# Maxwell-Zhao/RoboSimGS

Measured on AMD Instinct MI355X. Metric: frames/sec + ms/frame (fwd, fwd+bwd) at 1M Gaussians 1920x1080, higher is better.
Workload: dtype f32

## Files before the change

robosimgs_amd/csrc/build.py:

```python
from __future__ import annotations

import hashlib
import os
import shutil
import subprocess
import sys
from concurrent.futures import ThreadPoolExecutor

HERE = os.path.dirname(os.path.abspath(__file__))
SOURCES = ["api.hip", "projection.hip", "sort.hip", "binning.hip", "tile_sort.hip", "raster_fwd.hip",
           "raster_bwd.hip", "backward.hip", "composite.hip", "points.hip", "loss.hip", "transform.hip", "frame.hip"]
HEADERS = ["mgs_common.h", "mgs_math.h", "raster_common.h", "sh_staging.h", "tile_rect.h", "tile_order.h",
           "../../include/mgs.h"]
LIB = os.path.join(HERE, "libmgs.so")
DEBUG_LIB = os.path.join(HERE, "libmgs_debug.so")
HOOK_SOURCES = ["raster_fwd.hip", "sort.hip"]
OBJ_DIR = os.path.join(HERE, "build")
FLAGS = ["--offload-arch=gfx950", "-O3", "-std=c++17", "-fPIC", "-munsafe-fp-atomics",
         "-fno-slp-vectorize", "-Wall", "-Wno-unused-function"] + os.environ.get("MGS_EXTRA_FLAGS", "").split()


PER_SOURCE_FLAGS = {
    "raster_bwd.hip": os.environ.get("MGS_RASTER_BWD_FLAGS", "").split(),
    "raster_fwd.hip": os.environ.get("MGS_RASTER_FWD_FLAGS", "").split(),
    "tile_sort.hip": os.environ.get("MGS_TILE_SORT_FLAGS", "").split(),
    "binning.hip": os.environ.get("MGS_BINNING_FLAGS", "").split(),
}


def _hipcc() -> str:
    for c in (os.environ.get("HIPCC"), shutil.which("hipcc"), "/opt/rocm/bin/hipcc"):
        if c and os.path.exists(c):
            return c
    raise RuntimeError("hipcc not found; libmgs.so cannot be built")


def _stamp() -> str:
    h = hashlib.sha256((" ".join(FLAGS) + repr(sorted(PER_SOURCE_FLAGS.items()))).encode())
    for f in SOURCES + HEADERS:
        p = os.path.join(HERE, f)
        if os.path.exists(p):
            with open(p, "rb") as fh:
                h.update(fh.read())
    return h.hexdigest()


def _code_only(text: str) -> str:
    out, i, n = [], 0, len(text)
    while i < n:
        c = text[i]
        if c in "\"'":
            j = i + 1
            while j < n and text[j] != c:
                j += 2 if text[j] == "\\" else 1
            out.append(text[i:j + 1])
            i = j + 1
        elif text.startswith("//", i):
            j = text.find("\n", i)
            i = n if j < 0 else j
        elif text.startswith("/*", i):
            j = text.find("*/", i + 2)
            i = n if j < 0 else j + 2
            out.append(" ")
        else:
            out.append(c)
            i += 1
    return " ".join("".join(out).split())


def current_stamp() -> str:
    h = hashlib.sha256((" ".join(FLAGS) + repr(sorted(PER_SOURCE_FLAGS.items()))).encode())
    for f in SOURCES + HEADERS:
        p = os.path.join(HERE, f)
        if os.path.exists(p):
            with open(p, "r", encoding="utf-8", errors="replace") as fh:
                h.update(_code_only(fh.read()).encode())
    return h.hexdigest()


def build(force: bool = False, verbose: bool = False) -> str:
    stamp_file = os.path.join(OBJ_DIR, "stamp")
    stamp = _stamp()
    if (not force and os.path.exists(LIB) and os.path.exists(DEBUG_LIB) and os.path.exists(stamp_file)
            and open(stamp_file).read() == stamp):
        return LIB
    os.makedirs(OBJ_DIR, exist_ok=True)
    hipcc = _hipcc()
    srcs = [s for s in SOURCES if os.path.exists(os.path.join(HERE, s))]

    def compile_one(job) -> str:
        src, hooks = job
        obj = os.path.join(OBJ_DIR, src.replace(".hip", ".dbg.o" if hooks else ".o"))
        cmd = [hipcc, *FLAGS, *PER_SOURCE_FLAGS.get(src, []), *(["-DMGS_DEBUG_HOOKS"] if hooks else []), "-c",
               os.path.join(HERE, src), "-o", obj]
        if verbose:
            print(" ".join(cmd), flush=True)
        r = subprocess.run(cmd, capture_output=True, text=True)
        if r.returncode != 0:
            raise RuntimeError(f"hipcc failed on {src}:\n{r.stderr}")
# ... 21 lines not shown
```

robosimgs_amd/csrc/raster_bwd.hip:

```cpp
#include <algorithm>
#include <type_traits>

#include "raster_common.h"
#include "tile_order.h"

namespace mgs {
namespace {

template <int CHT, bool WIDE>
struct BwdEntry {
  float4 geo0;
  float4 geo1;
  float4 feat[(CHT + 3) / 4];
  float4 geo2;
  float4 geo3[WIDE ? 1 : 0];
};

template <int CHT>
struct BwdPixel {
  float T;
  float bv;
  float v_c[CHT];
  int last;
};

template <int CHT>
struct GaussGrad {
  float s, s_x, s_y, s_xx, s_xy, s_yy, a_x, a_y;
  float v_f[CHT];
};

template <int CHT, bool ABSGRAD, bool SAFE = false>
__device__ __forceinline__ void grad_pixel(BwdPixel<CHT>& px, GaussGrad<CHT>& gg, const PixelPoly& pp,
                                           float mx, float my, float ca, float cb,
                                           float cc, float A, float B, float C, float q0, float q1, float q2,
                                           const float* feat, int idx, int& any) {
  float ov = __builtin_amdgcn_exp2f(pair_power_poly(pp, q0, q1, q2, A, B, C));
  float alpha = SAFE ? ov : fminf(kAlphaMax, ov);
  bool valid = idx <= px.last && alpha >= kAlphaMin;
  if (!SAFE) valid = valid && pair_power_sign(mx - pp.x, my - pp.y, A, B, C) <= 0.f;
  if (ballot(valid) == 0ull) return;
  any = 1;
  float a_eff = valid ? alpha : 0.f;
  bool grad_geo = valid && ov <= kAlphaMax;
  float ov_eff = SAFE ? a_eff : (grad_geo ? ov : 0.f);
  float ra = __builtin_amdgcn_rcpf(1.0f - a_eff);
  px.T *= ra;
  float fac = a_eff * px.T;
  float fv = feat[0] * px.v_c[0];
#pragma unroll
  for (int c = 1; c < CHT; ++c) fv = fmaf(feat[c], px.v_c[c], fv);
  float v_alpha = fmaf(-px.bv, ra, fv * px.T);
  asm volatile("" : "+v"(px.bv), "+v"(v_alpha));
  px.bv = fmaf(fv, fac, px.bv);
#pragma unroll
  for (int c = 0; c < CHT; ++c) gg.v_f[c] = fmaf(fac, px.v_c[c], gg.v_f[c]);
  float v_sigma = -ov_eff * v_alpha;
  gg.s += v_sigma;
  gg.s_x = fmaf(v_sigma, pp.x, gg.s_x);
  gg.s_y = fmaf(v_sigma, pp.y, gg.s_y);
  gg.s_xx = fmaf(v_sigma, pp.xx, gg.s_xx);
  gg.s_xy = fmaf(v_sigma, pp.xy, gg.s_xy);
  gg.s_yy = fmaf(v_sigma, pp.yy, gg.s_yy);
  if (ABSGRAD) {
    float p = v_sigma * (mx - pp.x), q = v_sigma * (my - pp.y);
    gg.a_x += fabsf(fmaf(cb, q, ca * p));
    gg.a_y += fabsf(fmaf(cc, q, cb * p));
  }
}

__device__ __forceinline__ void moments_to_mean(float mx, float my, float s, float s_x, float s_y, float s_xx,
                                                float s_xy, float s_yy, float& P, float& Q, float& Vaa, float& Vab,
                                                float& Vbb) {
  P = fmaf(mx, s, -s_x);
  Q = fmaf(my, s, -s_y);
  Vaa = fmaf(mx, P, -fmaf(mx, s_x, -s_xx));
  Vab = fmaf(my, P, -fmaf(mx, s_y, -s_xy));
  Vbb = fmaf(my, Q, -fmaf(my, s_y, -s_yy));
}

__host__ __device__ constexpr int record_floats(int cht, bool absgrad) { return (6 + cht + (absgrad ? 2 : 0) + 3) / 4 * 4; }
__host__ __device__ constexpr int padded_channels(int channels) {
  return channels <= 4 ? channels : channels <= 8 ? 8 : channels <= 16 ? 16 : 32;
}

__device__ __forceinline__ void finish_geo(float ca, float cb, float cc, float& v_x, float& v_y,
                                           float& v_ca, float& v_cc) {
  const float s0 = v_x, s1 = v_y;
  v_x = fmaf(cb, s1, ca * s0);
  v_y = fmaf(cc, s1, cb * s0);
  v_ca *= 0.5f;
  v_cc *= 0.5f;
}

constexpr int kBwdMinWaves = 5;
constexpr int kBwdWgWaves = 1;
constexpr int kBwdXcdRun = 4;
#ifdef MGS_RASTER_BWD_TIMING
__device__ unsigned long long g_bwd_times[5 * 65536];
#endif
constexpr int kUnitClasses = 32;
struct UnitTables {
  uint32_t* counts;
  int4* whole;
  int4* part;
};
__host__ __device__ inline size_t unit_tables_bytes(int n_tiles, int shift, uint32_t capacity) {
  return 256 + (ckpt_units(capacity, n_tiles, shift) + (size_t)kUnitClasses * n_tiles) * sizeof(int4);
}
__device__ __forceinline__ UnitTables unit_tables(const int32_t* base, int n_tiles, int shift, uint32_t capacity) {
  UnitTables u;
  u.counts = reinterpret_cast<uint32_t*>(const_cast<int32_t*>(base));
  u.whole = reinterpret_cast<int4*>(const_cast<int32_t*>(base) + 64);
  u.part = u.whole + ckpt_units(capacity, n_tiles, shift);
  return u;
}

template <int CHT, bool ABSGRAD, bool RECORDS, bool SPLIT = false>
__device__ __forceinline__ void raster_bwd_unit(const int unit,
    const float* __restrict__ means2d, const float* __restrict__ conics,
    const float* __restrict__ feats, const float* __restrict__ opacities,
    const float4* __restrict__ splats, const float* __restrict__ background, int channels,
    int width, int height, int tile_w, int n_tiles, const int32_t* __restrict__ tile_offsets,
    const int32_t* __restrict__ flatten_ids, const float* __restrict__ alphas,
    const int32_t* __restrict__ last_ids, const float* __restrict__ v_render,
    const float* __restrict__ v_alphas, float* __restrict__ v_means2d,
    float* __restrict__ v_means2d_abs, float* __restrict__ v_conics,
    float* __restrict__ v_feats, float* __restrict__ v_opacities,
    const int4* __restrict__ pair_info, float* __restrict__ records,
    uint8_t* __restrict__ flags, uint32_t capacity, const float* __restrict__ expected_render,
    const int32_t* __restrict__ tile_order, const float* __restrict__ ckpt, int ckpt_shift,
    const int32_t* __restrict__ seg_table, const float* __restrict__ render_out, int splat_slots) {
  constexpr bool WIDE = ABSGRAD || !RECORDS;
  constexpr int NVR = 6 + CHT + (ABSGRAD ? 2 : 0);
  constexpr int kRedRows = !RECORDS ? 1 : (NVR > 8 && NVR <= 16) ? NVR : 8;
  __shared__ BwdEntry<CHT, WIDE> queues[kBwdWgWaves][kQueue];
  __shared__ float reds[kBwdWgWaves][kRedRows][64];
  BwdEntry<CHT, WIDE>* queue = queues[threadIdx.x >> 6];
  float (*red)[64] = reds[threadIdx.x >> 6];
  static_assert(!SPLIT || (RECORDS && CHT <= 4), "segments exist on the record path of up to 4 channels");
  constexpr int NQ = 4;
#ifdef MGS_RASTER_BWD_TIMING
  const unsigned long long t_enter = __builtin_amdgcn_s_memrealtime();
#endif
  int tile, seg = 0, seg_start = 0, seg_hi = 0;
  if constexpr (SPLIT) {
    const UnitTables ut = unit_tables(seg_table, n_tiles, ckpt_shift, capacity);
    uint32_t cnt[1 + kUnitClasses];
#pragma unroll
    for (int i = 0; i <= kUnitClasses; ++i) cnt[i] = ut.counts[i];
    const int4 e_whole = ut.whole[unit];
    int r = unit - (int)cnt[0], cls = -1, at = 0;
#pragma unroll
    for (int c = 0; c < kUnitClasses; ++c) {
      const int n = (int)cnt[1 + c];
      if (cls < 0 && r >= 0 && r < n) { cls = c; at = r; }
      if (r >= 0) r -= n;
    }
    if (r >= 0 && cls < 0) return;
    const int4 e = cls < 0 ? e_whole : ut.part[(size_t)cls * n_tiles + at];
    tile = e.x;
    seg = e.y;
    seg_start = e.z;
    seg_hi = e.w;
  } else {
    tile = tile_of_unit(unit, n_tiles, tile_order);
  }
  if (tile < 0) return;
  const unsigned lane = threadIdx.x & 63u;
  const int tx = tile % tile_w, ty = tile / tile_w;
  const float tile_x = (float)(tx * 16), tile_y = (float)(ty * 16);
  const int start = SPLIT ? seg_start : tile_offsets[tile], end = SPLIT ? seg_hi + 1 : tile_offsets[tile + 1];
  if (end <= start) return;
  const int lo = SPLIT ? start + (seg << ckpt_shift) : start;
  const int nxt = SPLIT ? lo + (1 << ckpt_shift) : end;
  if (RECORDS && capacity == 0u) return;
  const int ix = tx * 16 + (int)(lane & 7), iy = ty * 16 + (int)(lane >> 3);
  PixelPoly pq[NQ];
#pragma unroll
  for (int k = 0; k < NQ; ++k)
    pq[k] = pixel_poly((float)(lane & 7) - 7.5f + 8.f * (k & 1), (float)(int)(lane >> 3) - 7.5f + 8.f * (k >> 1));

  BwdPixel<CHT> st[NQ];
  int hi = -1;
  bool has_next = false;
  const float* cp = nullptr;
  if constexpr (SPLIT) {
    hi = seg_hi;
    if (hi < lo) return;
    has_next = hi >= nxt;
    cp = ckpt + ckpt_header_floats(n_tiles) + ckpt_unit(start, tile, seg + 1, ckpt_shift) * (size_t)(1 + channels) * 256 + lane;
    hi = min(hi, nxt - 1);
  }
  bool inside[NQ];
  float px_alpha[NQ], px_va[NQ], px_fin[NQ][CHT], px_ck[NQ][CHT + 1];
#pragma unroll
  for (int k = 0; k < NQ; ++k) {
    const int x = ix + 8 * (k & 1), y = iy + 8 * (k >> 1);
    inside[k] = x < width && y < height;
    const size_t p = inside[k] ? (size_t)y * width + x : 0;
    px_alpha[k] = inside[k] ? alphas[p] : 0.f;
    st[k].last = inside[k] ? last_ids[p] : -1;
    px_va[k] = (inside[k] && v_alphas) ? v_alphas[p] : 0.f;
    if (CHT == 4 && channels == 4) {
      const float4 v = inside[k] ? reinterpret_cast<const float4*>(v_render)[p] : make_float4(0.f, 0.f, 0.f, 0.f);
      st[k].v_c[0] = v.x; st[k].v_c[1 % CHT] = v.y; st[k].v_c[2 % CHT] = v.z; st[k].v_c[3 % CHT] = v.w;
    } else {
#pragma unroll
      for (int c = 0; c < CHT; ++c)
        st[k].v_c[c] = (inside[k] && c < channels) ? v_render[p * channels + c] : 0.f;
    }
    const float* frame = SPLIT ? (has_next ? render_out : expected_render) : expected_render;
#pragma unroll
    for (int c = 0; c < CHT; ++c) px_fin[k][c] = 0.f;
    if (frame && inside[k]) {
      if (CHT == 4 && channels == 4) {
        const float4 v = reinterpret_cast<const float4*>(frame)[p];
        px_fin[k][0] = v.x; px_fin[k][1 % CHT] = v.y; px_fin[k][2 % CHT] = v.z; px_fin[k][3 % CHT] = v.w;
      } else {
#pragma unroll
        for (int c = 0; c < CHT; ++c)
          if (c < channels && (SPLIT ? (has_next || c == channels - 1) : c == channels - 1)) px_fin[k][c] = frame[p * channels + c];
      }
    }
    if constexpr (SPLIT) {
#pragma unroll
      for (int c = 0; c <= CHT; ++c) px_ck[k][c] = (has_next && c <= channels) ? cp[256 * c + 64 * k] : 0.f;
    }
  }
#pragma unroll
  for (int k = 0; k < NQ; ++k) {
    st[k].T = 1.0f - px_alpha[k];
    float va = px_va[k];
    if (expected_render && inside[k]) {
      const float a = px_alpha[k], inv = 1.0f / fmaxf(a, 1e-10f);
#pragma unroll
      for (int c = 0; c < CHT; ++c)
        if (c == channels - 1) {
          const float v_ed = st[k].v_c[c];
          if (a > 1e-10f) va -= v_ed * px_fin[k][c] * inv;
          st[k].v_c[c] = v_ed * inv;
        }
    }
#pragma unroll
    for (int c = 0; c < CHT; ++c)
      if (background && c < channels) va -= background[c] * st[k].v_c[c];
    st[k].bv = -(st[k].T * va);
    if constexpr (SPLIT) {
      if (has_next && st[k].last >= nxt) {
        const float a = px_alpha[k], t_final = st[k].T;
        float behind = 0.f;
#pragma unroll
        for (int c = 0; c < CHT; ++c)
          if (c < channels) {
            float fin = px_fin[k][c];
            if (expected_render && c == channels - 1) fin *= fmaxf(a, 1e-10f);
            if (background) fin = fmaf(-t_final, background[c], fin);
            behind = fmaf(fin - px_ck[k][1 + c], st[k].v_c[c], behind);
          }
        st[k].bv += behind;
        st[k].T = px_ck[k][0];
      }
    } else {
      hi = max(hi, st[k].last);
    }
  }
  if constexpr (!SPLIT) {
#pragma unroll
    for (int d = 32; d >= 1; d >>= 1) hi = max(hi, __shfl_xor(hi, d));
    hi = min(hi, end - 1);
    if (hi < start) return;
  }
#ifdef MGS_RASTER_BWD_TIMING
  const unsigned long long t_begin = __builtin_amdgcn_s_memrealtime();
  unsigned long long n_walked = 0, n_pairs = 0;
#endif

  constexpr int NV = 6 + CHT + (ABSGRAD ? 2 : 0);
  constexpr int RSP = record_floats(CHT, ABSGRAD);
  auto rec_pos = [&](int j) { return j; };
  auto red_load = [&](float4& a0, float4& b0, float4& a1, float4& b1) {
    const int qv = (int)(lane >> 2), x = qv & 3;
    const float* q = &red[qv < NV ? qv : NV - 1][16 * (lane & 3)];
    a0 = *reinterpret_cast<const float4*>(q + 4 * x);
    b0 = *reinterpret_cast<const float4*>(q + 4 * (x ^ 1));
    a1 = *reinterpret_cast<const float4*>(q + 4 * (x ^ 2));
    b1 = *reinterpret_cast<const float4*>(q + 4 * (x ^ 3));
  };
  auto red_finish = [&](size_t rslot, const float4& a0, const float4& b0, const float4& a1, const float4& b1) {
    float t = (((a0.x + a0.y) + (a0.z + a0.w)) + ((b0.x + b0.y) + (b0.z + b0.w))) +
              (((a1.x + a1.y) + (a1.z + a1.w)) + ((b1.x + b1.y) + (b1.z + b1.w)));
    asm volatile("s_nop 1\n\tv_add_f32_dpp %0, %0, %0 quad_perm:[1,0,3,2] row_mask:0xf bank_mask:0xf\n\t"
                 "s_nop 1\n\tv_add_f32_dpp %0, %0, %0 quad_perm:[2,3,0,1] row_mask:0xf bank_mask:0xf" : "+v"(t));
    const float* rec = records + rslot * RSP;
    if ((lane & 3) == 0 && (int)(lane >> 2) < NV)
      asm volatile("global_store_dword %0, %1, %2" : : "v"((unsigned)(lane >> 2) * 4u), "v"(t), "s"(rec) : "memory");
    if (lane == 0) flags[rslot] = 1;
  };

  for (int q = (hi - start) / kQueue; q >= (lo - start) / kQueue; --q) {
    const int b = start + q * kQueue;
    unsigned live = 0;
#pragma unroll
    for (int k = 0; k < NQ; ++k)
      if (ballot(st[k].last >= b) != 0ull) live |= 1u << k;
    if (live == 0) continue;

    const int idx = b + (int)lane;
    unsigned qmask = 0;
    int g = 0;
    float2 xy = make_float2(0.f, 0.f);
    float ca = 1.f, cb = 0.f, cc = 1.f, op = 0.f;
    float pf[4] = {0.f, 0.f, 0.f, 0.f};
    uint32_t slot_base = 0u, slot_rect = 0u;
    const bool packed = CHT <= 4 && splats != nullptr;
    if (idx <= hi) {
      g = flatten_ids[idx];
      if (packed) {
        const float4 p0 = splats[3 * (size_t)g], p1 = splats[3 * (size_t)g + 1], p2 = splats[3 * (size_t)g + 2];
        xy = make_float2(p0.x, p0.y);
        ca = p0.z; cb = p0.w; cc = p1.x; op = p1.y;
        pf[0] = p1.z; pf[1] = p1.w; pf[2] = p2.x; pf[3] = p2.y;
        slot_base = __float_as_uint(p2.z); slot_rect = __float_as_uint(p2.w);
      } else {
        xy = reinterpret_cast<const float2*>(means2d)[g];
        ca = conics[3 * (size_t)g + 0];
        cb = conics[3 * (size_t)g + 1];
        cc = conics[3 * (size_t)g + 2];
        op = opacities[g];
      }
      qmask = quadrant_mask(xy.x, xy.y, ca, cb, cc, op, tile_x, tile_y);
      qmask &= live;
    }
    const unsigned long long keep = ballot(qmask != 0u);
    const int count = __popcll(keep);
#ifdef MGS_RASTER_BWD_TIMING
    n_walked += (unsigned long long)min(64, hi - b + 1);
    n_pairs += (unsigned long long)count;
#endif
    const bool all_safe = ballot(qmask != 0u && !entry_is_safe(ca, cb, cc, op)) == 0ull;
    if (qmask != 0u) {
      BwdEntry<CHT, WIDE>& e = queue[mask_rank(keep)];
      constexpr float kLog2e = 1.4426950408889634f;
      const float sA = -0.5f * kLog2e * ca, sB = -kLog2e * cb, sC = -0.5f * kLog2e * cc, L = __log2f(op);
      const float m_x = xy.x - (tile_x + 8.f), m_y = xy.y - (tile_y + 8.f);
      const PolyCoef pc = poly_coefs(m_x, m_y, sA, sB, sC, L);
      e.geo0 = make_float4(pc.q0, pc.q1, pc.q2, sA);
      e.geo1 = make_float4(sB, sC, __uint_as_float(qmask), __int_as_float(idx));
      int gid = g;
      if (RECORDS) {
        if (packed && splat_slots) {
          gid = (int)slot_base + (ty - (int)((slot_rect >> 10) & 1023u)) * (int)(slot_rect >> 20) + (tx - (int)(slot_rect & 1023u));
        } else {
          const int4 info = pair_info[g];
          gid = info.x + (ty - info.z) * (info.w & 0xffff) + (tx - info.y);
        }
      }
      e.geo2 = make_float4(__int_as_float(gid), m_x, m_y, L);
      if constexpr (WIDE) e.geo3[0] = make_float4(ca, cb, cc, 0.f);
      float f[((CHT + 3) / 4) * 4];
#pragma unroll
      for (int c = 0; c < ((CHT + 3) / 4) * 4; ++c)
        f[c] = (c < CHT && c < channels) ? (packed ? pf[c & 3] : feats[(size_t)g * channels + c]) : 0.f;
#pragma unroll
      for (int j = 0; j < (CHT + 3) / 4; ++j)
        e.feat[j] = make_float4(f[4 * j], f[4 * j + 1], f[4 * j + 2], f[4 * j + 3]);
    }
    __builtin_amdgcn_fence(__ATOMIC_RELEASE, "wavefront");
    __builtin_amdgcn_wave_barrier();
    __builtin_amdgcn_fence(__ATOMIC_ACQUIRE, "wavefront");

    auto walk = [&](auto safe_tag) {
    constexpr bool SAFE = decltype(safe_tag)::value;
    for (int j = count - 1; j >= 0; --j) {
      const BwdEntry<CHT, WIDE>& e = queue[j];
      const float4 g0 = e.geo0, g1 = e.geo1, g2 = e.geo2;
      float4 g3 = make_float4(0.f, 0.f, 0.f, 0.f);
      if constexpr (WIDE) g3 = e.geo3[0];
      float feat[CHT];
#pragma unroll
      for (int f = 0; f < (CHT + 3) / 4; ++f) {
        float4 v = e.feat[f];
        feat[4 * f] = v.x;
        if (4 * f + 1 < CHT) feat[4 * f + 1] = v.y;
        if (4 * f + 2 < CHT) feat[4 * f + 2] = v.z;
        if (4 * f + 3 < CHT) feat[4 * f + 3] = v.w;
      }
      const unsigned m = __builtin_amdgcn_readfirstlane(__float_as_uint(g1.z));
      const int gi = __float_as_int(g1.w);
      const int gid = __builtin_amdgcn_readfirstlane(__float_as_int(g2.x));
      GaussGrad<CHT> gg;
      gg.s = gg.s_x = gg.s_y = gg.s_xx = gg.s_xy = gg.s_yy = gg.a_x = gg.a_y = 0.f;
#pragma unroll
      for (int c = 0; c < CHT; ++c) gg.v_f[c] = 0.f;
      int any = 0;
#pragma unroll
      for (int k = 0; k < NQ; ++k) {
        if (m & (1u << k))
          grad_pixel<CHT, ABSGRAD, SAFE>(st[k], gg, pq[k], g2.y, g2.z, g3.x, g3.y, g3.z, g0.w, g1.x, g1.y,
                                         g0.x, g0.y, g0.z, feat, gi, any);
      }
      if (!any) continue;
      if constexpr (RECORDS) {
        if ((uint32_t)gid >= capacity) continue;
        const size_t rslot = (size_t)gid;
        float vals[NV];
        vals[0] = gg.s; vals[1] = gg.s_x; vals[2] = gg.s_y; vals[3] = gg.s_xx;
        vals[4] = gg.s_xy; vals[5] = gg.s_yy;
#pragma unroll
        for (int c = 0; c < CHT; ++c) vals[6 + c] = gg.v_f[c];
        if constexpr (ABSGRAD) { vals[6 + CHT] = gg.a_x; vals[7 + CHT] = gg.a_y; }
        int done = 0;
        if constexpr (NV > 8 && NV <= 16) {
#pragma unroll
          for (int i = 0; i < NV; ++i) red[i][lane] = vals[i];
          __builtin_amdgcn_fence(__ATOMIC_RELEASE, "wavefront");
          __builtin_amdgcn_wave_barrier();
          __builtin_amdgcn_fence(__ATOMIC_ACQUIRE, "wavefront");
          float4 a0, b0, a1, b1;
          red_load(a0, b0, a1, b1);
          red_finish(rslot, a0, b0, a1, b1);
          __builtin_amdgcn_wave_barrier();
          continue;
        }
        while (NV - done >= 8) {
#pragma unroll
          for (int i = 0; i < 8; ++i) red[i][lane] = vals[done + i];
          __builtin_amdgcn_fence(__ATOMIC_RELEASE, "wavefront");
          __builtin_amdgcn_wave_barrier();
          __builtin_amdgcn_fence(__ATOMIC_ACQUIRE, "wavefront");
          const float4* src = reinterpret_cast<const float4*>(&red[lane >> 3][(lane & 7) * 8]);
          const float4 a = src[0], b = src[1];
          float t = ((a.x + a.y) + (a.z + a.w)) + ((b.x + b.y) + (b.z + b.w));
          t += dpp_f(t, kDppXor1);
          t += dpp_f(t, kDppXor2);
          t += __int_as_float(__builtin_amdgcn_update_dpp(0, __float_as_int(t), 0x141, 0xf, 0xf, false));
          if ((lane & 7) == 0) {
            int pos = rec_pos(done + (int)(lane >> 3));
            if (pos >= 0) records[rslot * RSP + pos] = t;
          }
          __builtin_amdgcn_wave_barrier();
          done += 8;
        }
#define MGS_RS_CHUNK(V)                                                        \
        while (NV - done >= V) {                                               \
          float t = wave_reduce_scatter<V>(vals + done, lane);                 \
          int i = wave_reduce_scatter_index<V>(lane);                          \
          if (i >= 0) {                                                        \
            int pos = rec_pos(done + i);                                       \
            if (pos >= 0) records[rslot * RSP + pos] = t;                                        \
          }                                                                    \
          done += V;                                                           \
        }
        MGS_RS_CHUNK(4)
        MGS_RS_CHUNK(2)
        MGS_RS_CHUNK(1)
#undef MGS_RS_CHUNK
        if (lane == 0) flags[rslot] = 1;
      } else {
        const float ws = wave_reduce_to_lane63(gg.s), wx = wave_reduce_to_lane63(gg.s_x);
        const float wy = wave_reduce_to_lane63(gg.s_y), wxx = wave_reduce_to_lane63(gg.s_xx);
        const float wxy = wave_reduce_to_lane63(gg.s_xy), wyy = wave_reduce_to_lane63(gg.s_yy);
        float rx, ry, ra, rb, rc;
        moments_to_mean(g2.y, g2.z, ws, wx, wy, wxx, wxy, wyy, rx, ry, ra, rb, rc);
        const float ro = -ws * __builtin_amdgcn_exp2f(-g2.w);
        float rf[CHT];
#pragma unroll
        for (int c = 0; c < CHT; ++c) rf[c] = wave_reduce_to_lane63(gg.v_f[c]);
        float ax = 0.f, ay = 0.f;
        if (ABSGRAD) { ax = wave_reduce_to_lane63(gg.a_x); ay = wave_reduce_to_lane63(gg.a_y); }
        if (lane == 63) {
          finish_geo(g3.x, g3.y, g3.z, rx, ry, ra, rc);
          unsafeAtomicAdd(&v_means2d[2 * (size_t)gid + 0], rx);
          unsafeAtomicAdd(&v_means2d[2 * (size_t)gid + 1], ry);
          unsafeAtomicAdd(&v_conics[3 * (size_t)gid + 0], ra);
          unsafeAtomicAdd(&v_conics[3 * (size_t)gid + 1], rb);
          unsafeAtomicAdd(&v_conics[3 * (size_t)gid + 2], rc);
          unsafeAtomicAdd(&v_opacities[gid], ro);
#pragma unroll
          for (int c = 0; c < CHT; ++c)
            if (c < channels) unsafeAtomicAdd(&v_feats[(size_t)gid * channels + c], rf[c]);
          if (ABSGRAD) {
            unsafeAtomicAdd(&v_means2d_abs[2 * (size_t)gid + 0], ax);
            unsafeAtomicAdd(&v_means2d_abs[2 * (size_t)gid + 1], ay);
          }
        }
      }
    }
    };
    if (all_safe) walk(std::true_type{}); else walk(std::false_type{});
    __builtin_amdgcn_wave_barrier();
  }
#ifdef MGS_RASTER_BWD_TIMING
  if (lane == 0 && unit < 65536) {
    g_bwd_times[5 * unit + 0] = t_enter;
    g_bwd_times[5 * unit + 1] = t_begin;
    g_bwd_times[5 * unit + 2] = __builtin_amdgcn_s_memrealtime();
    g_bwd_times[5 * unit + 3] = n_walked;
    g_bwd_times[5 * unit + 4] = n_pairs;
  }
#endif
}

template <int CHT, bool ABSGRAD, bool RECORDS, bool SPLIT = false>
__global__ __launch_bounds__(64 * kBwdWgWaves, (CHT <= 4 && RECORDS && !ABSGRAD) ? kBwdMinWaves : 1) void raster_bwd_kernel(
    const float* __restrict__ means2d, const float* __restrict__ conics,
    const float* __restrict__ feats, const float* __restrict__ opacities,
    const float4* __restrict__ splats, const float* __restrict__ background, int channels,
    int width, int height, int tile_w, int n_tiles, const int32_t* __restrict__ tile_offsets,
    const int32_t* __restrict__ flatten_ids, const float* __restrict__ alphas,
    const int32_t* __restrict__ last_ids, const float* __restrict__ v_render,
    const float* __restrict__ v_alphas, float* __restrict__ v_means2d,
    float* __restrict__ v_means2d_abs, float* __restrict__ v_conics,
    float* __restrict__ v_feats, float* __restrict__ v_opacities,
    const int4* __restrict__ pair_info, float* __restrict__ records,
    uint8_t* __restrict__ flags, uint32_t capacity, const float* __restrict__ expected_render,
    const int32_t* __restrict__ tile_order, const float* __restrict__ ckpt, int ckpt_shift,
    const int32_t* __restrict__ seg_table, const float* __restrict__ render_out, int splat_slots) {
#define MGS_RB_ARGS means2d, conics, feats, opacities, splats, background, channels, width, height, tile_w, n_tiles, \
    tile_offsets, flatten_ids, alphas, last_ids, v_render, v_alphas, v_means2d, v_means2d_abs, v_conics, v_feats,    \
    v_opacities, pair_info, records, flags, capacity, expected_render, tile_order, ckpt, ckpt_shift, seg_table, render_out, splat_slots
  int unit = blockIdx.x * kBwdWgWaves + (int)(threadIdx.x >> 6);
  if constexpr (SPLIT && kBwdXcdRun > 1 && kBwdWgWaves == 1) {
    constexpr int R = kBwdXcdRun;
    const int b = unit, in = b % (8 * R);
    unit = b - in + (in & 7) * R + (in >> 3);
  }
  raster_bwd_unit<CHT, ABSGRAD, RECORDS, SPLIT>(unit, MGS_RB_ARGS);
#undef MGS_RB_ARGS
}

constexpr int kBigPairs = 256, kBigLists = 64, kBigWGs = 1024, kDiscoverPerThread = 16;
__host__ __device__ inline uint32_t big_list_room(uint32_t capacity) { return capacity / (uint32_t)kBigPairs + 1u; }
__host__ __device__ inline size_t big_lists_bytes(uint32_t capacity) { return (size_t)kBigLists * big_list_room(capacity) * sizeof(uint32_t); }

__device__ __forceinline__ void big_discover(int wg, int n, const int4* __restrict__ pair_info, uint32_t capacity,
                                             uint32_t* __restrict__ counts, uint32_t* __restrict__ items) {
  const int t = threadIdx.x;
  const uint32_t list = (uint32_t)(wg * 4 + (t >> 6)) % kBigLists, room = big_list_room(capacity);
  int4 info[kDiscoverPerThread];
#pragma unroll
  for (int j = 0; j < kDiscoverPerThread; ++j) {
    const int g = (wg * kDiscoverPerThread + j) * 256 + t;
    info[j] = g < n ? pair_info[g] : make_int4(0, 0, 0, 0);
  }
  unsigned long long mm[kDiscoverPerThread];
  uint32_t run[kDiscoverPerThread], wave_total = 0;
#pragma unroll
  for (int j = 0; j < kDiscoverPerThread; ++j) {
    mm[j] = ballot((info[j].w & 0xffff) * (int)((unsigned)info[j].w >> 16) >= kBigPairs);
    run[j] = wave_total;
    wave_total += (uint32_t)__popcll(mm[j]);
  }
  if (wave_total == 0u) return;
  uint32_t base = 0;
  if ((t & 63) == 0) base = atomicAdd(&counts[list], wave_total);
  base = __builtin_amdgcn_readfirstlane(base);
#pragma unroll
  for (int j = 0; j < kDiscoverPerThread; ++j) {
    const uint32_t at = base + run[j] + mask_rank(mm[j]);
    if (((mm[j] >> (t & 63)) & 1ull) && at < room) items[(size_t)list * room + at] = (uint32_t)((wg * kDiscoverPerThread + j) * 256 + t);
  }
}

__global__ __launch_bounds__(256) void unit_table_kernel(int n_tiles, const int32_t* __restrict__ tile_offsets,
                                                         const int32_t* __restrict__ tile_hi, int shift, uint32_t capacity,
                                                         int32_t* __restrict__ tables, int n, const int4* __restrict__ pair_info,
                                                         uint32_t* __restrict__ big_counts, uint32_t* __restrict__ big_items) {
  __shared__ uint32_t wave_tot[4], base, cls_n[kUnitClasses], cls_at[kUnitClasses];
  const int n_tile_wgs = (n_tiles + 255) / 256;
  if ((int)blockIdx.x >= n_tile_wgs) {
    big_discover((int)blockIdx.x - n_tile_wgs, n, pair_info, capacity, big_counts, big_items);
    return;
  }
  const UnitTables ut = unit_tables(tables, n_tiles, shift, capacity);
  const int tile = blockIdx.x * 256 + threadIdx.x, t = threadIdx.x;
  if (t < kUnitClasses) cls_n[t] = 0u;
  __syncthreads();
  int n_seg = 0, last_len = 0, u_start = 0, u_hi = 0;
  if (tile < n_tiles) {
    const int start = tile_offsets[tile], end = tile_offsets[tile + 1];
    const int4 h4 = reinterpret_cast<const int4*>(tile_hi)[tile];
    const int hi = min(max(max(h4.x, h4.y), max(h4.z, h4.w)), end - 1);
    u_start = start;
    u_hi = hi;
    if (hi >= start) {
      n_seg = ((hi - start) >> shift) + 1;
      last_len = ((hi - start) & ((1 << shift) - 1)) + 1;
    }
  }
  const uint32_t mine = n_seg > 0 ? (uint32_t)(n_seg - 1) : 0u;
  uint32_t incl = mine;
#pragma unroll
  for (int d = 1; d < 64; d <<= 1) {
    const uint32_t up = __shfl_up(incl, d);
    if ((t & 63) >= d) incl += up;
  }
  if ((t & 63) == 63) wave_tot[t >> 6] = incl;
  __syncthreads();
  uint32_t at = incl - mine;
  for (int w = 0; w < (t >> 6); ++w) at += wave_tot[w];
  const int c = n_seg > 0 ? ((1 << shift) - last_len) * kUnitClasses >> shift : 0;
  uint32_t rank = 0;
  if (n_seg > 0) rank = atomicAdd(&cls_n[c], 1u);
  if (t == 255) base = atomicAdd(&ut.counts[0], at + mine);
  __syncthreads();
  if (t < kUnitClasses && cls_n[t]) cls_at[t] = atomicAdd(&ut.counts[1 + t], cls_n[t]);
  __syncthreads();
  at += base;
  for (int sg = 0; sg + 1 < n_seg; ++sg) ut.whole[at + sg] = make_int4(tile, sg, u_start, u_hi);
  if (n_seg > 0) ut.part[(size_t)c * n_tiles + cls_at[c] + rank] = make_int4(tile, n_seg - 1, u_start, u_hi);
// ... 246 lines not shown
  float acc[NV];
#pragma unroll
  for (int i = 0; i < NV; ++i) acc[i] = 0.f;
  for (int base = 0; base < n_rows; base += 64) {
    const int t = base + lane;
    float rs[NV];
#pragma unroll
    for (int i = 0; i < NV; ++i) rs[i] = 0.f;
    if (t < n_rows) {
      int o = 0;
#pragma unroll
      for (int step = 32; step >= 1; step >>= 1)
        if (s_row0[wv][o + step] <= t) o += step;
      row_sum(s_info[wv][o], s_mean[wv][o], t - s_row0[wv][o], rs);
    }
#pragma unroll
    for (int i = 0; i < NV; ++i) s_rows[wv][lane * PITCH + i] = rs[i];
    __builtin_amdgcn_fence(__ATOMIC_RELEASE, "wavefront");
    __builtin_amdgcn_wave_barrier();
    __builtin_amdgcn_fence(__ATOMIC_ACQUIRE, "wavefront");
    const int a = max(row0, base), b = min(row0 + h, base + 64);
    for (int t2 = a; t2 < b; ++t2) {
#pragma unroll
      for (int i = 0; i < NV; ++i) acc[i] += s_rows[wv][(t2 - base) * PITCH + i];
    }
    __builtin_amdgcn_wave_barrier();
  }
  if (g >= n || is_big) return;
  if (h > 0) {
    finish_geo(ca, cb, cc, acc[0], acc[1], acc[2], acc[4]);
    acc[5] = op > 0.f ? -acc[5] / op : 0.f;
  }
  reinterpret_cast<float2*>(v_means2d)[g] = make_float2(acc[0], acc[1]);
  v_conics[3 * (size_t)g + 0] = acc[2];
  v_conics[3 * (size_t)g + 1] = acc[3];
  v_conics[3 * (size_t)g + 2] = acc[4];
  v_opacities[g] = acc[5];
#pragma unroll
  for (int c = 0; c < CHT; ++c)
    if (c < channels) v_feats[(size_t)g * channels + c] = acc[6 + c];
  if constexpr (ABSGRAD) reinterpret_cast<float2*>(v_means2d_abs)[g] = make_float2(acc[6 + CHT], acc[7 + CHT]);
}

struct BwdDetWs {
  size_t cap;
  int ckpt_shift = 0;
  size_t records, flags, big_counts, order, big_items, total;
  BwdDetWs(int channels, bool absgrad, uint32_t isect_capacity, int n_tiles, int checkpoint_interval)
      : cap(isect_capacity ? isect_capacity : 1) {
    while ((1 << ckpt_shift) < checkpoint_interval) ++ckpt_shift;
    Bump b(0);
    records = b.take(cap * record_floats(padded_channels(channels), absgrad) * sizeof(float));
    flags = b.take(cap);
    big_counts = b.take(256);
    static_assert(kBigLists * sizeof(uint32_t) <= 256, "the big lists' counters fit their header");
    order = b.take(std::max((size_t)n_tiles * sizeof(int32_t),
                            checkpoint_interval ? unit_tables_bytes(n_tiles, ckpt_shift, (uint32_t)cap) : 0));
    big_items = b.take(channels <= 4 ? big_lists_bytes((uint32_t)cap) : 0);
    total = b.total;
  }
};

}

size_t rasterize_bwd_det_workspace_bytes(int channels, bool absgrad, uint32_t capacity, int tile_w, int tile_h,
                                         int checkpoint_interval) {
  return BwdDetWs(channels, absgrad, capacity, tile_w * tile_h, checkpoint_interval).total;
}
}

using namespace mgs;

#ifdef MGS_RASTER_BWD_TIMING
extern "C" int mgs_debug_bwd_times(unsigned long long* host, int n_words) {
  hipError_t e = hipMemcpyFromSymbol(host, HIP_SYMBOL(g_bwd_times), (size_t)n_words * 8);
  if (e == hipSuccess) {
    void* dev = nullptr;
    e = hipGetSymbolAddress(&dev, HIP_SYMBOL(g_bwd_times));
    if (e == hipSuccess) e = hipMemset(dev, 0, sizeof(g_bwd_times));
  }
  return e == hipSuccess ? 0 : (int)e;
}
#endif
extern "C" int mgs_rasterize_bwd(int n, const float* means2d, const float* conics,
                                 const float* feats, const float* opacities,
                                 const float* background, int channels, int width, int height,
                                 int tile_w, int tile_h, const int32_t* tile_offsets,
                                 const int32_t* flatten_ids, const float* alphas,
                                 const int32_t* last_ids, const float* v_render,
                                 const float* v_alphas, float* v_means2d, float* v_means2d_abs,
                                 float* v_conics, float* v_feats, float* v_opacities,
                                 mgs_stream_t stream) {
  MGS_REQUIRE(n >= 0 && width > 0 && height > 0, "rasterize_bwd: bad sizes");
  MGS_REQUIRE(channels >= 1 && channels <= MGS_MAX_CHANNELS, "rasterize_bwd: channels %d outside 1..%d", channels, MGS_MAX_CHANNELS);
  MGS_REQUIRE(tile_w == (width + 15) / 16 && tile_h == (height + 15) / 16,
              "rasterize_bwd: tile grid does not match the image at tile size 16");
  if (n == 0) return MGS_OK;
  MGS_REQUIRE(means2d && conics && feats && opacities && tile_offsets && flatten_ids && alphas &&
                  last_ids && v_render && v_alphas && v_means2d && v_conics && v_feats &&
                  v_opacities, "rasterize_bwd: null pointer");
  const int n_tiles = tile_w * tile_h;
  hipStream_t s = (hipStream_t)stream;
  with_channels(channels, [&](auto cht) {
    with_bool(v_means2d_abs != nullptr, [&](auto absgrad) {
      hipLaunchKernelGGL((raster_bwd_kernel<decltype(cht)::value, decltype(absgrad)::value, false>),
                         dim3(div_up(n_tiles, kBwdWgWaves)), dim3(64 * kBwdWgWaves), 0, s, means2d, conics, feats, opacities,
                         (const float4*)nullptr, background, channels, width, height, tile_w, n_tiles, tile_offsets,
                         flatten_ids, alphas, last_ids, v_render, v_alphas, v_means2d, v_means2d_abs, v_conics, v_feats,
                         v_opacities, (const int4*)nullptr, (float*)nullptr, (uint8_t*)nullptr, 0u, (const float*)nullptr,
                         (const int32_t*)nullptr, (const float*)nullptr, 0, (const int32_t*)nullptr, (const float*)nullptr, 0);
    });
  });
  return check_launch("rasterize_bwd");
}

extern "C" int mgs_rasterize_bwd_det(int n, const float* means2d, const float* conics,
                                     const float* feats, const float* opacities,
                                     const float* splats, const float* background, int channels,
                                     int width,
                                     int height, int tile_w, int tile_h,
                                     const int32_t* tile_offsets, const int32_t* flatten_ids,
                                     const float* alphas, const int32_t* last_ids,
                                     const float* v_render, const float* v_alphas,
                                     const float* expected_render,
                                     const int32_t* pair_info, const int32_t* tile_group_order,
                                     uint32_t isect_capacity, const float* render_out,
                                     const float* checkpoints, int checkpoint_interval, int call_flags,
                                     float* v_means2d, float* v_means2d_abs, float* v_conics,
                                     float* v_feats, float* v_opacities, void* workspace,
                                     size_t* workspace_bytes, mgs_stream_t stream) {
  MGS_REQUIRE(n >= 0 && width > 0 && height > 0, "rasterize_bwd_det: bad sizes");
  MGS_REQUIRE(channels >= 1 && channels <= MGS_MAX_CHANNELS, "rasterize_bwd_det: channels %d outside 1..%d", channels, MGS_MAX_CHANNELS);
  MGS_REQUIRE(tile_w == (width + 15) / 16 && tile_h == (height + 15) / 16,
              "rasterize_bwd_det: tile grid does not match the image at tile size 16");
  MGS_REQUIRE(workspace_bytes, "rasterize_bwd_det: workspace_bytes is null");
  const bool split = checkpoints != nullptr && channels <= 4;
  if (checkpoints) {
    MGS_REQUIRE(checkpoint_interval >= 64 && (checkpoint_interval & (checkpoint_interval - 1)) == 0,
                "rasterize_bwd_det: checkpoint_interval %d is not a power of two >= 64", checkpoint_interval);
    MGS_REQUIRE(render_out, "rasterize_bwd_det: checkpoints need render_out (the forward's frame)");
    MGS_REQUIRE(!expected_render || expected_render == render_out, "rasterize_bwd_det: expected_render and render_out are the same frame");
  }
  const BwdDetWs ws(channels, v_means2d_abs != nullptr, isect_capacity, tile_w * tile_h, checkpoints ? checkpoint_interval : 0);
  const size_t cap = ws.cap, need = ws.total;
  const int ckpt_shift = ws.ckpt_shift;
  const size_t n_seg_units = checkpoints ? ckpt_units((uint32_t)cap, tile_w * tile_h, ckpt_shift) : 0;
  const bool big_path = channels <= 4;
  if (!workspace) {
    *workspace_bytes = need;
    return MGS_OK;
  }
  if (*workspace_bytes < need)
    return set_error(MGS_ERR_WORKSPACE_TOO_SMALL, "rasterize_bwd_det: workspace %zu < %zu bytes",
                     *workspace_bytes, need);
  if (n == 0) return MGS_OK;
  MGS_REQUIRE((reinterpret_cast<uintptr_t>(workspace) & 15u) == 0, "rasterize_bwd_det: workspace must be 16-byte aligned");
  MGS_REQUIRE(!splats || channels <= 4, "rasterize_bwd_det: packed splats carry at most 4 channels");
  MGS_REQUIRE(channels != 4 || (((reinterpret_cast<uintptr_t>(v_render) | reinterpret_cast<uintptr_t>(expected_render) |
                                  reinterpret_cast<uintptr_t>(render_out)) & 15u) == 0),
              "rasterize_bwd_det: 4-channel frames (v_render, expected_render, render_out) must be 16-byte aligned");
  const bool records_only = (call_flags & MGS_RASTER_BWD_RECORDS_ONLY) != 0;
  const int splat_slots = (call_flags & MGS_RASTER_BWD_SPLAT_SLOTS) != 0 ? 1 : 0;
  MGS_REQUIRE(!splat_slots || splats, "rasterize_bwd_det: MGS_RASTER_BWD_SPLAT_SLOTS needs the splat records");
  MGS_REQUIRE((splats || (means2d && conics && feats && opacities)) && tile_offsets && flatten_ids &&
                  alphas && last_ids && v_render && pair_info &&
                  (records_only || (v_means2d && v_conics && v_feats && v_opacities)), "rasterize_bwd_det: null pointer");
  const int n_tiles = tile_w * tile_h;
  hipStream_t s = (hipStream_t)stream;
  uint8_t* const w = static_cast<uint8_t*>(workspace);
  float* records = reinterpret_cast<float*>(w + ws.records);
  uint8_t* flags = w + ws.flags;
  uint32_t* big_counts = reinterpret_cast<uint32_t*>(w + ws.big_counts);
  uint32_t* big_items = reinterpret_cast<uint32_t*>(w + ws.big_items);
  hipError_t e = hipMemsetAsync(flags, 0, ws.order - ws.flags + (split ? 256 : 0), s);
  if (e != hipSuccess) return set_error((int)e, "rasterize_bwd_det: memset: %s", hipGetErrorString(e));
  const int4* info = reinterpret_cast<const int4*>(pair_info);
  const int32_t* order = nullptr;
  int32_t* seg_table = nullptr;
  if (split) {
    seg_table = reinterpret_cast<int32_t*>(w + ws.order);
    const unsigned n_disc = big_path && !records_only ? div_up(n, 256 * kDiscoverPerThread) : 0;
    hipLaunchKernelGGL(unit_table_kernel, dim3(div_up(n_tiles, 256) + n_disc), dim3(256), 0, s, n_tiles, tile_offsets,
                       reinterpret_cast<const int32_t*>(checkpoints), ckpt_shift, (uint32_t)cap, seg_table, n, info, big_counts, big_items);
  } else {
    order = tile_group_order;
    if (!order) {
      int32_t* mine = reinterpret_cast<int32_t*>(w + ws.order);
      const int rc = launch_tile_group_order(n_tiles, tile_offsets, mine, s);
      if (rc) return rc;
      order = mine;
    }
  }
  if (!split && big_path && !records_only)
    hipLaunchKernelGGL(big_discover_kernel, dim3(div_up(n, 256 * kDiscoverPerThread)), dim3(256), 0, s, n, info, (uint32_t)cap, big_counts, big_items);
  const int n_units = split ? (int)((n_seg_units + 8 * kBwdXcdRun - 1) / (8 * kBwdXcdRun)) * 8 * kBwdXcdRun
                            : order ? (n_tiles + 3) / 4 * 4 : n_tiles;
  with_channels(channels, [&](auto cht) {
    with_bool(v_means2d_abs != nullptr, [&](auto absgrad) {
      constexpr int C = decltype(cht)::value;
      constexpr bool A = decltype(absgrad)::value;
      auto raster = [&](auto seg) {
        hipLaunchKernelGGL((raster_bwd_kernel<C, A, true, decltype(seg)::value>), dim3(div_up(n_units, kBwdWgWaves)),
                           dim3(64 * kBwdWgWaves), 0, s, means2d, conics, feats, opacities,
                           reinterpret_cast<const float4*>(splats), background, channels, width, height, tile_w, n_tiles,
                           tile_offsets, flatten_ids, alphas, last_ids, v_render, v_alphas, (float*)nullptr, (float*)nullptr,
                           (float*)nullptr, (float*)nullptr, (float*)nullptr, info, records, flags, (uint32_t)cap,
                           expected_render, (const int32_t*)order, checkpoints, ckpt_shift, (const int32_t*)seg_table,
                           render_out, splat_slots);
      };
      if constexpr (C <= 4) with_bool(split, raster);
      else raster(bool_c<false>{});
      if (records_only) return;
      if constexpr (C <= 4)
        hipLaunchKernelGGL((reduce_records_rows_kernel<C, A>), dim3(kBigWGs + div_up(n, 256)), dim3(256), 0, s, n, info,
                           records, flags, (uint32_t)cap, means2d, conics, opacities, reinterpret_cast<const float4*>(splats),
                           channels, v_means2d, v_means2d_abs, v_conics, v_feats, v_opacities, big_counts, big_items);
      else
        hipLaunchKernelGGL((reduce_records_kernel<C, A>), dim3(div_up(n, 256)), dim3(256), 0, s, n, info, records, flags,
                           (uint32_t)cap, means2d, conics, opacities, reinterpret_cast<const float4*>(splats), channels,
                           v_means2d, v_means2d_abs, v_conics, v_feats, v_opacities);
    });
  });
  return check_launch("rasterize_bwd_det");
}
```

Before: 4375.

## Hand-write backward per-pixel gradient body in inline GCN assembly

Replaces the C++ per-pixel gradient accumulation in the backward rasterizer's safe path with inline gfx950 assembly for 3/4 channels. The assembly initializes the accumulators on the first hit instead of zeroing them, and uses exec-mask and ballot-precomputed started masks, with a separate variant for queues where some pixels end mid-batch. It also makes the tile coordinates scalar via readfirstlane and replaces the segment-entry select with a branch-free load. A debug hook keeps the C++ body selectable for comparison. The aim is fewer VALU instructions and less divergence in the hot loop, at the cost of fragile hand-written asm with manual exec handling.

```diff
diff --git a/robosimgs_amd/csrc/build.py b/robosimgs_amd/csrc/build.py
--- a/robosimgs_amd/csrc/build.py
+++ b/robosimgs_amd/csrc/build.py
@@ -14,7 +14,7 @@
            "../../include/mgs.h"]
 LIB = os.path.join(HERE, "libmgs.so")
 DEBUG_LIB = os.path.join(HERE, "libmgs_debug.so")
-HOOK_SOURCES = ["raster_fwd.hip", "sort.hip"]
+HOOK_SOURCES = ["raster_fwd.hip", "raster_bwd.hip", "sort.hip"]
 OBJ_DIR = os.path.join(HERE, "build")
 FLAGS = ["--offload-arch=gfx950", "-O3", "-std=c++17", "-fPIC", "-munsafe-fp-atomics",
          "-fno-slp-vectorize", "-Wall", "-Wno-unused-function"] + os.environ.get("MGS_EXTRA_FLAGS", "").split()
diff --git a/robosimgs_amd/csrc/raster_bwd.hip b/robosimgs_amd/csrc/raster_bwd.hip
--- a/robosimgs_amd/csrc/raster_bwd.hip
+++ b/robosimgs_amd/csrc/raster_bwd.hip
@@ -69,6 +69,101 @@
   }
 }
 
+template <int CHT>
+__device__ __forceinline__ void grad_pixel_safe_asm(BwdPixel<CHT>& px, GaussGrad<CHT>& gg, const PixelPoly& pp,
+                                                    float A, float B, float C, float q0, float q1, float q2,
+                                                    const float* feat, unsigned long long started, unsigned& init) {
+  static_assert(CHT == 3 || CHT == 4, "hand-written backward body: 3 or 4 channels");
+  float t1, r, fv, va;
+  const float amin = kAlphaMin;
+#define MGS_BWD_BODY(FV3, VF3_MUL, VF3_FMAC)                                                                         \
+      "v_fma_f32 %[t1], %[q1], %[x], %[q0]\n"                                       \
+      "v_fmac_f32 %[t1], %[q2], %[y]\n"                                                                              \
+      "v_fmac_f32 %[t1], %[A], %[xx]\n"                                                                              \
+      "v_fmac_f32 %[t1], %[B], %[xy]\n"                                                                              \
+      "v_fmac_f32 %[t1], %[C], %[yy]\n"                                                                              \
+      "v_exp_f32 %[t1], %[t1]\n"                                                                                     \
+      "v_mul_f32 %[fv], %[c0], %[f0]\n"                                       \
+      "s_cmp_lg_u32 %[init], 0\n"                                                                                    \
+      "s_cbranch_scc1 .Lmgs_bwd_acc%=\n"                                                                             \
+                                                               \
+      "v_cmp_le_f32 vcc, %[amin], %[t1]\n"                                                                           \
+      "s_and_b64 vcc, vcc, %[started]\n"                                    \
+      "s_cbranch_scc0 .Lmgs_bwd_end%=\n"                                                                             \
+      "s_mov_b32 %[init], 1\n"                                                                                       \
+      "v_cndmask_b32 %[t1], 0, %[t1], vcc\n"                                                              \
+      "v_sub_f32 %[r], 1.0, %[t1]\n"                                                                                 \
+      "v_rcp_f32 %[r], %[r]\n"                                                                                       \
+      "v_fmac_f32 %[fv], %[f1], %[c1]\n"                                                                             \
+      "v_fmac_f32 %[fv], %[f2], %[c2]\n"                                                                             \
+      FV3                                                                                                            \
+      "v_mul_f32 %[T], %[T], %[r]\n"                                                                                 \
+      "v_mul_f32 %[va], %[T], %[fv]\n"                                                                               \
+      "v_fma_f32 %[va], -%[bv], %[r], %[va]\n"                                                          \
+      "v_mul_f32 %[r], %[t1], %[T]\n"                                                                       \
+      "v_fmac_f32 %[bv], %[fv], %[r]\n"                                                                              \
+      "v_mul_f32 %[vf0], %[r], %[c0]\n"                                                                              \
+      "v_mul_f32 %[vf1], %[r], %[c1]\n"                                                                              \
+      "v_mul_f32 %[vf2], %[r], %[c2]\n"                                                                              \
+      VF3_MUL                                                                                                        \
+      "v_mul_f32 %[s], %[va], -%[t1]\n"                                                                 \
+      "v_mul_f32 %[sx], %[s], %[x]\n"                                                                                \
+      "v_mul_f32 %[sy], %[s], %[y]\n"                                                                                \
+      "v_mul_f32 %[sxx], %[s], %[xx]\n"                                                                              \
+      "v_mul_f32 %[sxy], %[s], %[xy]\n"                                                                              \
+      "v_mul_f32 %[syy], %[s], %[yy]\n"                                                                              \
+      "s_branch .Lmgs_bwd_end%=\n"                                                                                   \
+                                                        \
+      ".Lmgs_bwd_acc%=:\n"                                                                                           \
+      "s_mov_b64 exec, %[started]\n"                                                                                 \
+      "v_cmpx_le_f32 vcc, %[amin], %[t1]\n"                                                                          \
+      "s_cbranch_execz .Lmgs_bwd_out%=\n"                                                                            \
+      "v_sub_f32 %[r], 1.0, %[t1]\n"                                                                                 \
+      "v_rcp_f32 %[r], %[r]\n"                                                                                       \
+      "v_fmac_f32 %[fv], %[f1], %[c1]\n"                                                                             \
+      "v_fmac_f32 %[fv], %[f2], %[c2]\n"                                                                             \
+      FV3                                                                                                            \
+      "v_mul_f32 %[T], %[T], %[r]\n"                                                                                 \
+      "v_mul_f32 %[va], %[T], %[fv]\n"                                                                               \
+      "v_fma_f32 %[va], -%[bv], %[r], %[va]\n"                                                                       \
+      "v_mul_f32 %[r], %[t1], %[T]\n"                                                                                \
+      "v_fmac_f32 %[bv], %[fv], %[r]\n"                                                                              \
+      "v_fmac_f32 %[vf0], %[r], %[c0]\n"                                                                             \
+      "v_fmac_f32 %[vf1], %[r], %[c1]\n"                                                                             \
+      "v_fmac_f32 %[vf2], %[r], %[c2]\n"                                                                             \
+      VF3_FMAC                                                                                                       \
+      "v_mul_f32 %[fv], %[va], -%[t1]\n"                                                                             \
+      "v_fma_f32 %[s], %[va], -%[t1], %[s]\n"                                                                        \
+      "v_fmac_f32 %[sx], %[fv], %[x]\n"                                                                              \
+      "v_fmac_f32 %[sy], %[fv], %[y]\n"                                                                              \
+      "v_fmac_f32 %[sxx], %[fv], %[xx]\n"                                                                            \
+      "v_fmac_f32 %[sxy], %[fv], %[xy]\n"                                                                            \
+      "v_fmac_f32 %[syy], %[fv], %[yy]\n"                                                                            \
+      ".Lmgs_bwd_out%=:\n"                                                                                           \
+      "s_mov_b64 exec, -1\n"                                                                                         \
+      ".Lmgs_bwd_end%=:\n"
+#define MGS_BWD_OUT                                                                                                  \
+      [t1] "=&v"(t1), [r] "=&v"(r), [fv] "=&v"(fv), [va] "=&v"(va), [T] "+v"(px.T), [bv] "+v"(px.bv),              \
+      [s] "+v"(gg.s), [sx] "+v"(gg.s_x), [sy] "+v"(gg.s_y), [sxx] "+v"(gg.s_xx), [sxy] "+v"(gg.s_xy),               \
+      [syy] "+v"(gg.s_yy), [vf0] "+v"(gg.v_f[0]), [vf1] "+v"(gg.v_f[1]), [vf2] "+v"(gg.v_f[2]), [init] "+s"(init)
+#define MGS_BWD_IN                                                                                                   \
+      [q0] "v"(q0), [q1] "v"(q1), [q2] "v"(q2), [x] "v"(pp.x), [y] "v"(pp.y), [xx] "v"(pp.xx), [xy] "v"(pp.xy),      \
+      [yy] "v"(pp.yy), [A] "v"(A), [B] "v"(B), [C] "v"(C), [f0] "v"(feat[0]), [f1] "v"(feat[1]), [f2] "v"(feat[2]),  \
+      [c0] "v"(px.v_c[0]), [c1] "v"(px.v_c[1]), [c2] "v"(px.v_c[2]), [amin] "s"(amin), [started] "s"(started)
+  if constexpr (CHT == 4) {
+    asm volatile(MGS_BWD_BODY("v_fmac_f32 %[fv], %[f3], %[c3]\n", "v_mul_f32 %[vf3], %[r], %[c3]\n",
+                              "v_fmac_f32 %[vf3], %[r], %[c3]\n")
+                 : MGS_BWD_OUT, [vf3] "+v"(gg.v_f[3])
+                 : MGS_BWD_IN, [f3] "v"(feat[3]), [c3] "v"(px.v_c[3])
+                 : "vcc", "scc");
+  } else {
+    asm volatile(MGS_BWD_BODY("", "", "") : MGS_BWD_OUT : MGS_BWD_IN : "vcc", "scc");
+  }
+#undef MGS_BWD_BODY
+#undef MGS_BWD_OUT
+#undef MGS_BWD_IN
+}
+
 __device__ __forceinline__ void moments_to_mean(float mx, float my, float s, float s_x, float s_y, float s_xx,
                                                 float s_xy, float s_yy, float& P, float& Q, float& Vaa, float& Vab,
                                                 float& Vbb) {
@@ -116,7 +211,7 @@
   return u;
 }
 
-template <int CHT, bool ABSGRAD, bool RECORDS, bool SPLIT = false>
+template <int CHT, bool ABSGRAD, bool RECORDS, bool SPLIT = false, bool CXX_BODY = false>
 __device__ __forceinline__ void raster_bwd_unit(const int unit,
     const float* __restrict__ means2d, const float* __restrict__ conics,
     const float* __restrict__ feats, const float* __restrict__ opacities,
@@ -140,6 +235,7 @@
   float (*red)[64] = reds[threadIdx.x >> 6];
   static_assert(!SPLIT || (RECORDS && CHT <= 4), "segments exist on the record path of up to 4 channels");
   constexpr int NQ = 4;
+  constexpr bool kAsmBody = (CHT == 3 || CHT == 4) && RECORDS && !ABSGRAD && !CXX_BODY;
 #ifdef MGS_RASTER_BWD_TIMING
   const unsigned long long t_enter = __builtin_amdgcn_s_memrealtime();
 #endif
@@ -158,18 +254,19 @@
       if (r >= 0) r -= n;
     }
     if (r >= 0 && cls < 0) return;
-    const int4 e = cls < 0 ? e_whole : ut.part[(size_t)cls * n_tiles + at];
-    tile = e.x;
-    seg = e.y;
-    seg_start = e.z;
-    seg_hi = e.w;
+    const int4 e_part = ut.part[(size_t)max(cls, 0) * n_tiles + at];
+    tile = cls < 0 ? e_whole.x : e_part.x;
+    seg = cls < 0 ? e_whole.y : e_part.y;
+    seg_start = cls < 0 ? e_whole.z : e_part.z;
+    seg_hi = cls < 0 ? e_whole.w : e_part.w;
   } else {
     tile = tile_of_unit(unit, n_tiles, tile_order);
   }
   if (tile < 0) return;
   const unsigned lane = threadIdx.x & 63u;
-  const int tx = tile % tile_w, ty = tile / tile_w;
-  const float tile_x = (float)(tx * 16), tile_y = (float)(ty * 16);
+  const int tx = __builtin_amdgcn_readfirstlane(tile % tile_w), ty = __builtin_amdgcn_readfirstlane(tile / tile_w);
+  const float tile_x = __int_as_float(__builtin_amdgcn_readfirstlane(__float_as_int((float)(tx * 16))));
+  const float tile_y = __int_as_float(__builtin_amdgcn_readfirstlane(__float_as_int((float)(ty * 16))));
   const int start = SPLIT ? seg_start : tile_offsets[tile], end = SPLIT ? seg_hi + 1 : tile_offsets[tile + 1];
   if (end <= start) return;
   const int lo = SPLIT ? start + (seg << ckpt_shift) : start;
@@ -301,9 +398,12 @@
   for (int q = (hi - start) / kQueue; q >= (lo - start) / kQueue; --q) {
     const int b = start + q * kQueue;
     unsigned live = 0;
-#pragma unroll
-    for (int k = 0; k < NQ; ++k)
-      if (ballot(st[k].last >= b) != 0ull) live |= 1u << k;
+    unsigned long long reach[NQ];
+#pragma unroll
+    for (int k = 0; k < NQ; ++k) {
+      reach[k] = ballot(st[k].last >= b);
+      if (reach[k] != 0ull) live |= 1u << k;
+    }
     if (live == 0) continue;
 
     const int idx = b + (int)lane;
@@ -314,6 +414,8 @@
     float pf[4] = {0.f, 0.f, 0.f, 0.f};
     uint32_t slot_base = 0u, slot_rect = 0u;
     const bool packed = CHT <= 4 && splats != nullptr;
+    float btx = tile_x, bty = tile_y;
+    asm volatile("" : "+v"(btx), "+v"(bty));
     if (idx <= hi) {
       g = flatten_ids[idx];
       if (packed) {
@@ -329,7 +431,7 @@
         cc = conics[3 * (size_t)g + 2];
         op = opacities[g];
       }
-      qmask = quadrant_mask(xy.x, xy.y, ca, cb, cc, op, tile_x, tile_y);
+      qmask = quadrant_mask(xy.x, xy.y, ca, cb, cc, op, btx, bty);
       qmask &= live;
     }
     const unsigned long long keep = ballot(qmask != 0u);
@@ -339,6 +441,16 @@
     n_pairs += (unsigned long long)count;
 #endif
     const bool all_safe = ballot(qmask != 0u && !entry_is_safe(ca, cb, cc, op)) == 0ull;
+    unsigned long long full[NQ];
+    bool mixed = false;
+    if constexpr (kAsmBody) {
+      const int hb = min(b + kQueue - 1, hi);
+#pragma unroll
+      for (int k = 0; k < NQ; ++k) {
+        full[k] = ballot(st[k].last >= hb);
+        mixed = mixed || (reach[k] & ~full[k]) != 0ull;
+      }
+    }
     if (qmask != 0u) {
       BwdEntry<CHT, WIDE>& e = queue[mask_rank(keep)];
       constexpr float kLog2e = 1.4426950408889634f;
@@ -370,8 +482,9 @@
     __builtin_amdgcn_wave_barrier();
     __builtin_amdgcn_fence(__ATOMIC_ACQUIRE, "wavefront");
 
-    auto walk = [&](auto safe_tag) {
+    auto walk = [&](auto safe_tag, auto mixed_tag) {
     constexpr bool SAFE = decltype(safe_tag)::value;
+    constexpr bool MIXED = decltype(mixed_tag)::value;
     for (int j = count - 1; j >= 0; --j) {
       const BwdEntry<CHT, WIDE>& e = queue[j];
       const float4 g0 = e.geo0, g1 = e.geo1, g2 = e.geo2;
@@ -390,15 +503,27 @@
       const int gi = __float_as_int(g1.w);
       const int gid = __builtin_amdgcn_readfirstlane(__float_as_int(g2.x));
       GaussGrad<CHT> gg;
-      gg.s = gg.s_x = gg.s_y = gg.s_xx = gg.s_xy = gg.s_yy = gg.a_x = gg.a_y = 0.f;
-#pragma unroll
-      for (int c = 0; c < CHT; ++c) gg.v_f[c] = 0.f;
       int any = 0;
-#pragma unroll
-      for (int k = 0; k < NQ; ++k) {
-        if (m & (1u << k))
-          grad_pixel<CHT, ABSGRAD, SAFE>(st[k], gg, pq[k], g2.y, g2.z, g3.x, g3.y, g3.z, g0.w, g1.x, g1.y,
-                                         g0.x, g0.y, g0.z, feat, gi, any);
+      if constexpr (kAsmBody && SAFE) {
+        unsigned init = 0u;
+#pragma unroll
+        for (int k = 0; k < NQ; ++k) {
+          if (m & (1u << k)) {
+            const unsigned long long started = MIXED ? ballot(gi <= st[k].last) : full[k];
+            grad_pixel_safe_asm<CHT>(st[k], gg, pq[k], g0.w, g1.x, g1.y, g0.x, g0.y, g0.z, feat, started, init);
+          }
+        }
+        any = (int)init;
+      } else {
+        gg.s = gg.s_x = gg.s_y = gg.s_xx = gg.s_xy = gg.s_yy = gg.a_x = gg.a_y = 0.f;
+#pragma unroll
+        for (int c = 0; c < CHT; ++c) gg.v_f[c] = 0.f;
+#pragma unroll
+        for (int k = 0; k < NQ; ++k) {
+          if (m & (1u << k))
+            grad_pixel<CHT, ABSGRAD, SAFE>(st[k], gg, pq[k], g2.y, g2.z, g3.x, g3.y, g3.z, g0.w, g1.x, g1.y,
+                                           g0.x, g0.y, g0.z, feat, gi, any);
+        }
       }
       if (!any) continue;
       if constexpr (RECORDS) {
@@ -488,7 +613,13 @@
       }
     }
     };
-    if (all_safe) walk(std::true_type{}); else walk(std::false_type{});
+    if (!all_safe) {
+      walk(std::false_type{}, std::false_type{});
+    } else if constexpr (kAsmBody) {
+      if (mixed) walk(std::true_type{}, std::true_type{}); else walk(std::true_type{}, std::false_type{});
+    } else {
+      walk(std::true_type{}, std::false_type{});
+    }
     __builtin_amdgcn_wave_barrier();
   }
 #ifdef MGS_RASTER_BWD_TIMING
@@ -502,7 +633,7 @@
 #endif
 }
 
-template <int CHT, bool ABSGRAD, bool RECORDS, bool SPLIT = false>
+template <int CHT, bool ABSGRAD, bool RECORDS, bool SPLIT = false, bool CXX_BODY = false>
 __global__ __launch_bounds__(64 * kBwdWgWaves, (CHT <= 4 && RECORDS && !ABSGRAD) ? kBwdMinWaves : 1) void raster_bwd_kernel(
     const float* __restrict__ means2d, const float* __restrict__ conics,
     const float* __restrict__ feats, const float* __restrict__ opacities,
@@ -526,7 +657,7 @@
     const int b = unit, in = b % (8 * R);
     unit = b - in + (in & 7) * R + (in >> 3);
   }
-  raster_bwd_unit<CHT, ABSGRAD, RECORDS, SPLIT>(unit, MGS_RB_ARGS);
+  raster_bwd_unit<CHT, ABSGRAD, RECORDS, SPLIT, CXX_BODY>(unit, MGS_RB_ARGS);
 #undef MGS_RB_ARGS
 }
 
@@ -939,6 +1070,11 @@
   return e == hipSuccess ? 0 : (int)e;
 }
 #endif
+#ifdef MGS_DEBUG_HOOKS
+static int g_raster_bwd_body = 0;
+extern "C" void mgs_debug_set_raster_bwd_body(int body) { g_raster_bwd_body = body; }
+#endif
+
 extern "C" int mgs_rasterize_bwd(int n, const float* means2d, const float* conics,
                                  const float* feats, const float* opacities,
                                  const float* background, int channels, int width, int height,
@@ -1057,13 +1193,24 @@
       constexpr int C = decltype(cht)::value;
       constexpr bool A = decltype(absgrad)::value;
       auto raster = [&](auto seg) {
-        hipLaunchKernelGGL((raster_bwd_kernel<C, A, true, decltype(seg)::value>), dim3(div_up(n_units, kBwdWgWaves)),
-                           dim3(64 * kBwdWgWaves), 0, s, means2d, conics, feats, opacities,
-                           reinterpret_cast<const float4*>(splats), background, channels, width, height, tile_w, n_tiles,
-                           tile_offsets, flatten_ids, alphas, last_ids, v_render, v_alphas, (float*)nullptr, (float*)nullptr,
-                           (float*)nullptr, (float*)nullptr, (float*)nullptr, info, records, flags, (uint32_t)cap,
-                           expected_render, (const int32_t*)order, checkpoints, ckpt_shift, (const int32_t*)seg_table,
-                           render_out, splat_slots);
+        auto launch = [&](auto cxx_body) {
+          hipLaunchKernelGGL((raster_bwd_kernel<C, A, true, decltype(seg)::value, decltype(cxx_body)::value>),
+                             dim3(div_up(n_units, kBwdWgWaves)), dim3(64 * kBwdWgWaves), 0, s, means2d, conics, feats,
+                             opacities, reinterpret_cast<const float4*>(splats), background, channels, width, height, tile_w,
+                             n_tiles, tile_offsets, flatten_ids, alphas, last_ids, v_render, v_alphas, (float*)nullptr,
+                             (float*)nullptr, (float*)nullptr, (float*)nullptr, (float*)nullptr, info, records, flags,
+                             (uint32_t)cap, expected_render, (const int32_t*)order, checkpoints, ckpt_shift,
+                             (const int32_t*)seg_table, render_out, splat_slots);
+        };
+#ifdef MGS_DEBUG_HOOKS
+        if constexpr ((C == 3 || C == 4) && !A) {
+          if (g_raster_bwd_body == 1) {
+            launch(bool_c<true>{});
+            return;
+          }
+        }
+#endif
+        launch(bool_c<false>{});
       };
       if constexpr (C <= 4) with_bool(split, raster);
       else raster(bool_c<false>{});
```

Result: no change. 4388 (median of 6 runs) (+0.3%).
